# borglab/gtsfm

Hardware: NVIDIA H100
Metric: image_pairs_per_sec (higher is better)
Workload: dtype f32

## Files before the change

gtsfm_b200/_lib.py:

```python
from __future__ import annotations

import ctypes as C
from pathlib import Path
from typing import Optional

import numpy as np

LIB_PATH = Path(__file__).resolve().parent / "libgtsfm_b200.so"

_lib: Optional[C.CDLL] = None


class B200Error(RuntimeError):
    pass


class LightGlueParams(C.Structure):
    _fields_ = [("depth_confidence", C.c_double), ("width_confidence", C.c_double), ("filter_threshold", C.c_double),
                ("prune_min_kpts", C.c_int), ("fp16_attention", C.c_int)]


class LightGluePair(C.Structure):
    _fields_ = [("kp0", C.c_void_p), ("desc0", C.c_void_p), ("n0", C.c_int), ("kp1", C.c_void_p), ("desc1", C.c_void_p), ("n1", C.c_int),
                ("out_matches", C.c_void_p), ("out_scores", C.c_void_p), ("out_k", C.c_int), ("out_stop_layer", C.c_int)]


class MnnPair(C.Structure):
    _fields_ = [("desc0", C.c_void_p), ("n0", C.c_int), ("desc1", C.c_void_p), ("n1", C.c_int), ("out_matches", C.c_void_p),
                ("out_dist", C.c_void_p), ("out_k", C.c_int)]


MNN_ERR_RATIO = -4


class SiftKeypoint(C.Structure):
    _fields_ = [("x", C.c_float), ("y", C.c_float), ("size", C.c_float), ("angle", C.c_float), ("response", C.c_float),
                ("octave", C.c_int32)]


SIFT_KEYPOINT_DTYPE = np.dtype([("x", np.float32), ("y", np.float32), ("size", np.float32), ("angle", np.float32),
                                ("response", np.float32), ("octave", np.int32)])


class SiftImage(C.Structure):
    _fields_ = [("image", C.c_void_p), ("mask", C.c_void_p), ("max_keypoints", C.c_int), ("out_keypoints", C.c_void_p),
                ("out_desc", C.c_void_p), ("out_n", C.c_int), ("out_total", C.c_int)]


SIFT_CAPACITY = -5


class RansacParams(C.Structure):
    _fields_ = [("threshold", C.c_double), ("confidence", C.c_double), ("max_iters", C.c_int), ("seed", C.c_uint64)]


_vp, _i, _f, _sz = C.c_void_p, C.c_int, C.c_float, C.c_size_t
_ip = C.POINTER(C.c_int)

SIGNATURES = {
    "b2_version": (_i, []),
    "b2_create": (_i, [_i, C.POINTER(_vp)]),
    "b2_destroy": (None, [_vp]),
    "b2_last_error": (C.c_char_p, [_vp]),
    "b2_launch_count": (C.c_uint64, [_vp]),
    "b2_h2d_bytes": (C.c_uint64, [_vp]),
    "b2_set_option": (C.c_int, [_vp, C.c_char_p, C.c_int64]),
    "b2_profile_start": (_i, [_vp, C.c_char_p]),
    "b2_profile_stop": (_i, [_vp, C.POINTER(C.c_double), C.POINTER(C.c_uint64), C.POINTER(C.c_double)]),
    "b2_debug_fetch": (C.c_int64, [_vp, C.c_char_p, _vp, C.c_int64]),
    "b2_debug_gemm_host": (_i, [_vp, _i, _vp, _vp, _vp, _vp, _i, _i, _i]),
    "b2_superpoint_set_weights": (_i, [_vp, _vp, _sz]),
    "b2_superpoint_detect_dev": (_i, [_vp, _vp, _i, _i, _i, _sz, _f, _i, _i, _vp, _vp, _i, _ip, C.POINTER(C.c_uint64), _vp]),
    "b2_superpoint_describe_dev": (_i, [_vp, C.c_uint64, _vp, _i, _vp, _vp]),
    "b2_superpoint_extract_dev": (_i, [_vp, _vp, _i, _i, _i, _sz, _f, _i, _i, _i, _vp, _vp, _vp, _ip, _vp]),
    "b2_superpoint_extract_async_dev": (_i, [_vp, _vp, _i, _i, _i, _sz, _f, _i, _i, _i, _vp, _vp, _vp, _vp, _vp]),
    "b2_superpoint_finish_dev": (_i, [_vp, _vp]),
    "b2_topk_indices_dev": (_i, [_vp, _vp, _i, _i, _vp, _ip, _vp]),
    "b2_superpoint_detect_host": (_i, [_vp, _vp, _i, _i, _i, _f, _i, _i, _vp, _vp, _i, _ip, C.POINTER(C.c_uint64)]),
    "b2_superpoint_describe_host": (_i, [_vp, C.c_uint64, _vp, _i, _vp]),
    "b2_image_resize_dev": (_i, [_vp, _vp, _i, _i, _i, _sz, _vp, _i, _i, _vp]),
    "b2_lightglue_set_weights": (_i, [_vp, _vp, _sz]),
    "b2_lightglue_match_dev": (_i, [_vp, _vp, _vp, _i, _vp, _vp, _i, C.POINTER(LightGlueParams), _vp, _vp, _ip, _ip, _vp]),
    "b2_lightglue_match_host": (_i, [_vp, _vp, _vp, _i, _vp, _vp, _i, C.POINTER(LightGlueParams), _vp, _vp, _ip, _ip]),
    "b2_lightglue_match_batched_dev": (_i, [_vp, C.POINTER(LightGluePair), _i, C.POINTER(LightGlueParams), _vp]),
    "b2_superglue_set_weights": (_i, [_vp, _vp, _sz]),
    "b2_superglue_match_dev": (_i, [_vp, _vp, _vp, _vp, _i, _i, _i, _vp, _vp, _vp, _i, _i, _i, _i, _f, _vp, _vp, _ip, _vp]),
    "b2_superglue_match_host": (_i, [_vp, _vp, _vp, _vp, _i, _i, _i, _vp, _vp, _vp, _i, _i, _i, _i, _f, _vp, _vp, _ip]),
    "b2_netvlad_blob_floats": (_sz, []),
    "b2_netvlad_set_weights": (_i, [_vp, _vp, _sz]),
    "b2_netvlad_describe_dev": (_i, [_vp, _vp, _i, _i, _i, _vp, _vp]),
    "b2_netvlad_describe_host": (_i, [_vp, _vp, _i, _i, _i, _vp]),
    "b2_megaloc_blob_floats": (_sz, []),
    "b2_megaloc_set_weights": (_i, [_vp, _vp, _sz]),
    "b2_megaloc_describe_dev": (_i, [_vp, _vp, _i, _i, _i, _vp, _vp]),
    "b2_megaloc_describe_host": (_i, [_vp, _vp, _i, _i, _i, _vp]),
    "b2_megaloc_describe_u8_dev": (_i, [_vp, _vp, _i, _i, _i, _sz, _vp, _vp]),
    "b2_megaloc_resize_u8_dev": (_i, [_vp, _vp, _i, _i, _i, _sz, _vp, _vp]),
    "b2_similarity_pairs_host": (_i, [_vp, _vp, _i, _i, _i, _f, _vp, _vp]),
    "b2_ransac_essential_host": (_i, [_vp, _vp, _vp, _i, C.POINTER(RansacParams), _vp, _vp, _ip, _vp, _vp]),
    "b2_ransac_fundamental_host": (_i, [_vp, _vp, _vp, _i, C.POINTER(RansacParams), _vp, _vp, _ip]),
    "b2_ransac_essential_dev": (_i, [_vp, _vp, _vp, _vp, _i, _vp, _vp, C.POINTER(RansacParams), _vp, _vp, _ip, _vp, _vp, _vp]),
    "b2_recover_pose_host": (_i, [_vp, _vp, _vp, _vp, _i, _vp, _vp, _ip]),
    "b2_mnn_match_batched_dev": (_i, [_vp, C.POINTER(MnnPair), _i, _i, _i, C.c_double, _vp]),
    "b2_mnn_match_host": (_i, [_vp, _vp, _i, _vp, _i, _i, _i, C.c_double, _vp, _vp, _ip]),
    "b2_sift_detect_batched_dev": (_i, [_vp, C.POINTER(SiftImage), _i, _i, _i, _i, _sz, _vp]),
    "b2_sift_detect_host": (_i, [_vp, _vp, _i, _i, _i, _vp, _vp, _vp, _i, _ip]),
}


def load() -> C.CDLL:
    global _lib
    if _lib is not None:
        return _lib
    if not LIB_PATH.exists():
        raise B200Error(f"{LIB_PATH} is missing: run `python -m gtsfm_b200.build` (there is no CPU fallback)")
    lib = C.CDLL(str(LIB_PATH))
    for name, (res, args) in SIGNATURES.items():
        fn = getattr(lib, name)
        fn.restype = res
        fn.argtypes = args
    _lib = lib
    return lib


def ptr(a) -> C.c_void_p:
    if a is None:
        return C.c_void_p(0)
    if isinstance(a, np.ndarray):
        assert a.flags["C_CONTIGUOUS"], "array must be C-contiguous"
        return C.c_void_p(a.ctypes.data)
    if hasattr(a, "data_ptr"):
        assert a.is_contiguous(), "tensor must be contiguous"
        return C.c_void_p(a.data_ptr())
    return C.c_void_p(int(a))


class Context:

    def __init__(self, device: int = 0):
        self._lib = load()
        h = C.c_void_p()
        rc = self._lib.b2_create(int(device), C.byref(h))
        if rc != 0 or not h:
            raise B200Error(
                f"b2_create(device={device}) failed with {rc}: an sm_90 (H100) GPU is required; there is no CPU fallback")
        self.handle = h
        self.device = device

    def check(self, rc: int, what: str) -> None:
        if rc < 0:
            raise B200Error(f"{what} failed ({rc}): {self._lib.b2_last_error(self.handle).decode()}")

    @property
# ... 37 lines not shown
```

gtsfm_b200/csrc/attn_ps.cuh:

```cuda
#pragma once
#include "tma.cuh"

constexpr int AW_Q = 128, AW_KV = 64, AW_D = 64;
constexpr int AW_KV_BYTES = AW_KV * AW_D * 2;
constexpr int AS_NS = 4;
constexpr int AS_HALF = 2 * AW_KV_BYTES;
constexpr int AS_STAGE = 2 * AS_HALF;
constexpr int AS_TILE_BYTES = AS_NS * AS_STAGE;
constexpr int AS_Q_PLANE = AW_Q * AW_D * 2;
constexpr int AS_Q_BYTES = 2 * 2 * AS_Q_PLANE;
constexpr size_t AS_SMEM = AS_TILE_BYTES + AS_Q_BYTES + 1024 + 512;
constexpr int AS_THREADS = 256 + 32;
constexpr float AS_RESCALE = 8.0f;
constexpr int AP_MAXP = 16;

struct AttnPsMaps {
  CUtensorMap kh[AP_MAXP], kl[AP_MAXP], vh[AP_MAXP], vl[AP_MAXP];
};

struct AttnPsProblem {
  const __half *Qh, *Ql;
  __half *Oh, *Ol;
  int Nq, Nk;
  int ldo;
  int qt, tiles;
  int w_end;
  int item0;
};
struct AttnPsArgs {
  AttnPsProblem p[AP_MAXP];
  int nprob;
  float* Opart;
  float* ml;
  int* arrivals;
  int W;
  int quota;
  int max_splits;
  float scale;
  int* err_flag;
};

struct AttnPsSeg {
  int z, item, h, q0, tile0, T, split, nsplits, itemg;
};
__device__ __forceinline__ AttnPsSeg attn_ps_decode(const AttnPsArgs& a, int w, int w_end) {
  AttnPsSeg s;
  s.z = 0;
  while (s.z + 1 < a.nprob && w >= a.p[s.z].w_end) ++s.z;
  const AttnPsProblem& p = a.p[s.z];
  const int base = s.z ? a.p[s.z - 1].w_end : 0;
  const int wl = w - base;
  s.item = wl / p.tiles;
  s.tile0 = wl - s.item * p.tiles;
  s.T = min(p.tiles - s.tile0, w_end - w);
  s.h = s.item / p.qt;
  s.q0 = (s.item - s.h * p.qt) * (2 * AW_Q);
  const int wi0 = base + s.item * p.tiles, wi1 = wi0 + p.tiles;
  const int c_first = wi0 / a.quota;
  s.split = w / a.quota - c_first;
  s.nsplits = (wi1 - 1) / a.quota - c_first + 1;
  s.itemg = p.item0 + s.item;
  return s;
}

template <bool SINGLE>
static __global__ void __launch_bounds__(AS_THREADS, 1) k_flash_ps(const __grid_constant__ AttnPsMaps maps, const __grid_constant__ AttnPsArgs args) {
  extern __shared__ unsigned char ap_raw[];
  const uint32_t raw = tc::smem_u32(ap_raw);
  const uint32_t smem0 = (raw + 1023u) & ~1023u;
  unsigned char* sm = ap_raw + (smem0 - raw);
  uint64_t* bars = reinterpret_cast<uint64_t*>(sm + AS_TILE_BYTES + AS_Q_BYTES);
  uint64_t* kv_full = bars;
  uint64_t* kv_empty = kv_full + AS_NS;
  volatile int* last_flag = reinterpret_cast<volatile int*>(kv_empty + AS_NS);

  const int t = threadIdx.x, warp = t >> 5, lane = t & 31;
  const int w_begin = blockIdx.x * args.quota;
  const int w_end = min(args.W, w_begin + args.quota);

  if (t == 0) {
    for (int i = 0; i < AS_NS; ++i) tc::mbar_init(&kv_full[i], 1), tc::mbar_init(&kv_empty[i], 8);
    tc::fence_mbar_init();
  }
  __syncthreads();
  bool ok = true;

  if (warp == 8) {
    if (lane == 0) {
      int ge = 0;
      for (int w = w_begin; w < w_end;) {
        const AttnPsSeg sg = attn_ps_decode(args, w, w_end);
        const int Nk = args.p[sg.z].Nk;
        for (int e = 0; e < sg.T + 2; ++e) {
          const int g = ge + e, s = g % AS_NS;
          if (g >= AS_NS) ok = tc::mbar_wait(&kv_empty[s], ((g / AS_NS) - 1) & 1) && ok;
          const bool hk = e < sg.T, hv = e >= 2;
          constexpr int PART = SINGLE ? AW_KV_BYTES : AS_HALF;
          tc::mbar_expect_tx(&kv_full[s], (hk ? PART : 0) + (hv ? PART : 0));
          const uint32_t dst = smem0 + s * AS_STAGE;
          if (hk) {
            const int row = sg.h * Nk + (sg.tile0 + e) * AW_KV;
            tc::tma_load_2d(dst, &maps.kh[sg.z], &kv_full[s], 0, row);
            if (!SINGLE) tc::tma_load_2d(dst + AW_KV_BYTES, &maps.kl[sg.z], &kv_full[s], 0, row);
          }
          if (hv) {
            const int row = sg.h * Nk + (sg.tile0 + e - 2) * AW_KV;
            tc::tma_load_2d(dst + AS_HALF, &maps.vh[sg.z], &kv_full[s], 0, row);
            if (!SINGLE) tc::tma_load_2d(dst + AS_HALF + AW_KV_BYTES, &maps.vl[sg.z], &kv_full[s], 0, row);
          }
        }
        ge += sg.T + 2;
        w += sg.T;
      }
    }
  } else {
    const int q = warp >> 2;
    const int r = t & 127;
    const int rq = (warp & 3) * 16 + (lane >> 2);
    const int c2 = (lane & 3) * 2;
    const uint32_t sQ = smem0 + AS_TILE_BYTES + q * 2 * AS_Q_PLANE;
    const float c2s = args.scale * 1.4426950408889634f;
    auto wg_bar = [&]() { asm volatile("bar.sync %0, 128;" ::"r"(1 + q) : "memory"); };
    auto release = [&](int g) { if (lane == 0) tc::mbar_arrive(&kv_empty[g % AS_NS]); };

    int ge = 0;
    for (int w = w_begin; w < w_end;) {
      const AttnPsSeg sg = attn_ps_decode(args, w, w_end);
      const AttnPsProblem& pr = args.p[sg.z];
      const int T = sg.T, Nk = pr.Nk;
      {
        const int qrow = sg.q0 + q * AW_Q + r;
        wg_bar();
#pragma unroll
        for (int pl = 0; pl < (SINGLE ? 1 : 2); ++pl) {
          const __half* src = (pl ? pr.Ql : pr.Qh) + ((size_t)sg.h * pr.Nq + qrow) * 64;
          unsigned char* dst = sm + AS_TILE_BYTES + q * 2 * AS_Q_PLANE + pl * AS_Q_PLANE + r * 128;
#pragma unroll
          for (int c = 0; c < 8; ++c) {
            uint4 v = make_uint4(0u, 0u, 0u, 0u);
            if (qrow < pr.Nq) v = __ldg(reinterpret_cast<const uint4*>(src) + c);
            *reinterpret_cast<uint4*>(dst + ((c ^ (r & 7)) << 4)) = v;
          }
        }
        tc::fence_proxy_async();
        wg_bar();
      }
      float o[2][32];
      float m_ref[2][2], l_i[2][2];
#pragma unroll
      for (int sl = 0; sl < 2; ++sl)
#pragma unroll
        for (int h = 0; h < 2; ++h) m_ref[sl][h] = -INFINITY, l_i[sl][h] = 0.f;
      for (int j = 0; j < 2; ++j) ok = tc::mbar_wait(&kv_full[(ge + j) % AS_NS], ((ge + j) / AS_NS) & 1) && ok;
      if (T == 1) release(ge + 1);
      for (int i = 0; i < T; ++i) {
        const int gv = ge + i + 2;
        ok = tc::mbar_wait(&kv_full[gv % AS_NS], (gv / AS_NS) & 1) && ok;
        const uint32_t sK = smem0 + ((ge + i) % AS_NS) * AS_STAGE, sV = smem0 + (gv % AS_NS) * AS_STAGE + AS_HALF;
        const uint64_t dKh = tc::wg_desc_sw128(sK), dKl = tc::wg_desc_sw128(sK + AW_KV_BYTES);
        const uint64_t dVh = tc::wg_desc_sw128(sV), dVl = tc::wg_desc_sw128(sV + AW_KV_BYTES);
        const int k0 = (sg.tile0 + i) * AW_KV;
#pragma unroll
        for (int sl = 0; sl < 2; ++sl) {
          const uint64_t dQh = tc::wg_desc_sw128(sQ + sl * (64 * 128)), dQl = tc::wg_desc_sw128(sQ + AS_Q_PLANE + sl * (64 * 128));
          float a[32];
          tc::wg_fence();
#pragma unroll
          for (int ks = 0; ks < 4; ++ks) {
            const uint64_t adv = (uint64_t)(ks * 2);
            tc::wg_ss_n64(a, dQh + adv, dKh + adv, ks ? 1u : 0u);
            if (!SINGLE) {
              tc::wg_ss_n64(a, dQh + adv, dKl + adv, 1u);
              tc::wg_ss_n64(a, dQl + adv, dKh + adv, 1u);
            }
          }
          tc::wg_commit();
          tc::wg_wait<0>();
          if (k0 + AW_KV > Nk) {
#pragma unroll
            for (int jj = 0; jj < 32; ++jj)
              if (k0 + 8 * (jj >> 2) + c2 + (jj & 1) >= Nk) a[jj] = -INFINITY;
          }
          uint32_t ph[16], pl[16];
#pragma unroll
          for (int h = 0; h < 2; ++h) {
            float mx = a[2 * h];
#pragma unroll
            for (int j = 0; j < 8; ++j) mx = fmaxf(mx, fmaxf(a[4 * j + 2 * h], a[4 * j + 2 * h + 1]));
            mx = fmaxf(mx, __shfl_xor_sync(0xffffffffu, mx, 1));
            mx = fmaxf(mx, __shfl_xor_sync(0xffffffffu, mx, 2));
            const float m_new = fmaxf(m_ref[sl][h], mx * c2s);
            if (m_new - m_ref[sl][h] > AS_RESCALE) {
              const float corr = tc::ex2(m_ref[sl][h] - m_new);
              l_i[sl][h] *= corr;
              if (i > 0) {
#pragma unroll
                for (int j = 0; j < 8; ++j) o[sl][4 * j + 2 * h] *= corr, o[sl][4 * j + 2 * h + 1] *= corr;
              }
              m_ref[sl][h] = m_new;
            }
            float rs = 0.f;
#pragma unroll
            for (int j = 0; j < 8; ++j) {
              const float p0 = tc::ex2(fmaf(a[4 * j + 2 * h], c2s, -m_ref[sl][h]));
              const float p1 = tc::ex2(fmaf(a[4 * j + 2 * h + 1], c2s, -m_ref[sl][h]));
              rs += p0 + p1;
              const __half2 hh = __floats2half2_rn(p0, p1);
              const int ri = 4 * (j >> 1) + 2 * (j & 1) + h;
              ph[ri] = *reinterpret_cast<const uint32_t*>(&hh);
              if (!SINGLE) {
                const float2 hf = __half22float2(hh);
                const __half2 ll = __floats2half2_rn(p0 - hf.x, p1 - hf.y);
                pl[ri] = *reinterpret_cast<const uint32_t*>(&ll);
              }
            }
            l_i[sl][h] += rs;
          }
          tc::wg_fence();
#pragma unroll
          for (int ks = 0; ks < 4; ++ks) {
            const uint64_t advV = (uint64_t)(ks * 128);
            tc::wg_rs_n64_bt(o[sl], ph + 4 * ks, dVh + advV, (i | ks) ? 1u : 0u);
            if (!SINGLE) {
              tc::wg_rs_n64_bt(o[sl], ph + 4 * ks, dVl + advV, 1u);
              tc::wg_rs_n64_bt(o[sl], pl + 4 * ks, dVh + advV, 1u);
            }
          }
          tc::wg_commit();
          tc::wg_wait<0>();
        }
        release(ge + i);
        if (i + 2 >= T) release(gv);
      }
      ge += T + 2;
      w += T;
#pragma unroll
      for (int sl = 0; sl < 2; ++sl)
#pragma unroll
        for (int h = 0; h < 2; ++h) {
          l_i[sl][h] += __shfl_xor_sync(0xffffffffu, l_i[sl][h], 1);
          l_i[sl][h] += __shfl_xor_sync(0xffffffffu, l_i[sl][h], 2);
        }
      auto write_row = [&](const float* v, float inv, int qrow) {
        uint32_t* dh = reinterpret_cast<uint32_t*>(pr.Oh + (size_t)qrow * pr.ldo + sg.h * 64 + c2);
        uint32_t* dl = reinterpret_cast<uint32_t*>(pr.Ol + (size_t)qrow * pr.ldo + sg.h * 64 + c2);
#pragma unroll
        for (int j = 0; j < 8; ++j) {
          uint32_t hi, lo;
          if (SINGLE) {
            const __half2 hh = __floats2half2_rn(tc::clamp_h(v[4 * j] * inv), tc::clamp_h(v[4 * j + 1] * inv));
            hi = *reinterpret_cast<const uint32_t*>(&hh), lo = 0u;
          } else {
            tc::split2(v[4 * j] * inv, v[4 * j + 1] * inv, hi, lo);
          }
          dh[4 * j] = hi;
          dl[4 * j] = lo;
        }
      };
      if (sg.nsplits == 1) {
#pragma unroll
        for (int sl = 0; sl < 2; ++sl)
#pragma unroll
          for (int h = 0; h < 2; ++h) {
            const int qrow = sg.q0 + q * AW_Q + sl * 64 + rq + 8 * h;
            if (qrow >= pr.Nq) continue;
            float v[32];
#pragma unroll
            for (int j = 0; j < 8; ++j) v[4 * j] = o[sl][4 * j + 2 * h], v[4 * j + 1] = o[sl][4 * j + 2 * h + 1];
            write_row(v, 1.0f / l_i[sl][h], qrow);
          }
      } else {
        const size_t slot0 = (size_t)sg.itemg * args.max_splits;
#pragma unroll
        for (int sl = 0; sl < 2; ++sl)
#pragma unroll
          for (int h = 0; h < 2; ++h) {
            const int rl = q * AW_Q + sl * 64 + rq + 8 * h;
            if (sg.q0 + rl >= pr.Nq) continue;
            const size_t rowi = (slot0 + sg.split) * 256 + rl;
            float* dst = args.Opart + rowi * 64 + c2;
#pragma unroll
            for (int j = 0; j < 8; ++j) *reinterpret_cast<float2*>(dst + 8 * j) = make_float2(o[sl][4 * j + 2 * h], o[sl][4 * j + 2 * h + 1]);
            if (c2 == 0) *reinterpret_cast<float2*>(args.ml + rowi * 2) = make_float2(m_ref[sl][h], l_i[sl][h]);
          }
        __threadfence();
        wg_bar();
        if (r == 0) {
          int* cnt = args.arrivals + sg.itemg * 2 + q;
          const int old = atomicAdd(cnt, 1);
          const int last = old == sg.nsplits - 1;
          if (last) atomicExch(cnt, 0);
          last_flag[q] = last;
        }
        wg_bar();
        if (last_flag[q]) {
          __threadfence();
#pragma unroll 1
          for (int sl = 0; sl < 2; ++sl)
#pragma unroll 1
            for (int h = 0; h < 2; ++h) {
              const int rl = q * AW_Q + sl * 64 + rq + 8 * h;
              const int qrow = sg.q0 + rl;
              if (qrow >= pr.Nq) continue;
              float m = -INFINITY;
              for (int sp = 0; sp < sg.nsplits; ++sp) m = fmaxf(m, __ldcg(args.ml + ((slot0 + sp) * 256 + rl) * 2));
              float l = 0.f, v[32];
#pragma unroll
              for (int j = 0; j < 32; ++j) v[j] = 0.f;
              for (int sp = 0; sp < sg.nsplits; ++sp) {
                const size_t ri = (slot0 + sp) * 256 + rl;
                const float2 mlv = __ldcg(reinterpret_cast<const float2*>(args.ml + ri * 2));
                const float wgt = tc::ex2(mlv.x - m);
                l = fmaf(mlv.y, wgt, l);
                const float* src = args.Opart + ri * 64 + c2;
// ... 15 lines not shown
```

gtsfm_b200/csrc/debug.cu:

```cuda
#include <stdlib.h>

#include "common.cuh"
#include "linear.cuh"

extern "C" int b2_debug_gemm_host(b2_context* ctx, int mode, const float* A, const float* B, const float* bias, float* C,
                                  int M, int N, int K) {
  if (!ctx || !A || !B || !C || M <= 0 || N <= 0 || K <= 0 || (K % 64)) return B2_ERR_ARG;
  std::lock_guard<std::mutex> lk(ctx->mu);
  cudaSetDevice(ctx->device);
  cudaStream_t st = ctx->stream;
  DevBuf dA, dB, dC, dBias, dBh, dBl, dErr;
  B2_CUDA(ctx, dA.ensure((size_t)M * K * 4));
  B2_CUDA(ctx, dB.ensure((size_t)N * K * 4));
  B2_CUDA(ctx, dC.ensure((size_t)M * N * 4));
  B2_CUDA(ctx, dBias.ensure((size_t)N * 4));
  B2_CUDA(ctx, dErr.ensure(16));
  B2_CUDA(ctx, cudaMemcpyAsync(dA.p, A, (size_t)M * K * 4, cudaMemcpyHostToDevice, st));
  B2_CUDA(ctx, cudaMemcpyAsync(dB.p, B, (size_t)N * K * 4, cudaMemcpyHostToDevice, st));
  if (bias) B2_CUDA(ctx, cudaMemcpyAsync(dBias.p, bias, (size_t)N * 4, cudaMemcpyHostToDevice, st));
  B2_CUDA(ctx, cudaMemsetAsync(dErr.p, 0, 16, st));
  int rc = B2_OK;
  if (mode == 0) {
    rc = launch_gemm(ctx, st, gemm_linear(dA.as<float>(), K, K, dB.as<float>(), bias ? dBias.as<float>() : nullptr, dC.as<float>(), N, M, N));
  } else {
    DevBuf dAh, dAl;
    B2_CUDA(ctx, dAh.ensure((size_t)M * K * 2));
    B2_CUDA(ctx, dAl.ensure((size_t)M * K * 2));
    B2_CUDA(ctx, dBh.ensure((size_t)N * K * 2));
    B2_CUDA(ctx, dBl.ensure((size_t)N * K * 2));
    B2_LAUNCH(ctx, k_split_f32, (unsigned)(((size_t)M * K + 255) / 256), 256, 0, st, dA.as<float>(), (size_t)M * K, dAh.as<__half>(), dAl.as<__half>());
    B2_LAUNCH(ctx, k_split_f32, (unsigned)(((size_t)N * K + 255) / 256), 256, 0, st, dB.as<float>(), (size_t)N * K, dBh.as<__half>(), dBl.as<__half>());
    B2_CUDA(ctx, cudaFuncSetAttribute(k_gemm_ws, cudaFuncAttributeMaxDynamicSharedMemorySize, (int)GW_SMEM));
    TcWeights tw{nullptr, nullptr, nullptr, dErr.as<int>(), true};
    tw.sm_count = ctx->sm_count;
    LinArgs a;
    a.a1p = {dAh.as<__half>(), dAl.as<__half>()}, a.lda1 = K, a.K1 = K, a.bp = {dBh.as<__half>(), dBl.as<__half>()}, a.ldb = K;
    a.bias = bias ? dBias.as<float>() : nullptr, a.cf = dC.as<float>(), a.ldc = N, a.tc_want_f32 = true, a.M = M, a.N = N;
    rc = run_linear(ctx, st, tw, &a, 1);
    if (rc == B2_OK) {
      cudaError_t e = cudaStreamSynchronize(st);
      if (e != cudaSuccess) rc = b2_fail(ctx, B2_ERR_CUDA, std::string("debug gemm: ") + cudaGetErrorString(e));
    }
    dAh.release(), dAl.release();
  }
  int err = 0;
  if (rc == B2_OK) {
    cudaError_t e = cudaMemcpyAsync(C, dC.p, (size_t)M * N * 4, cudaMemcpyDeviceToHost, st);
    if (e == cudaSuccess) e = cudaMemcpyAsync(&err, dErr.p, 4, cudaMemcpyDeviceToHost, st);
    if (e == cudaSuccess) e = cudaStreamSynchronize(st);
    if (e != cudaSuccess) rc = b2_fail(ctx, B2_ERR_CUDA, std::string("debug gemm: ") + cudaGetErrorString(e));
  }
  dA.release(), dB.release(), dC.release(), dBias.release(), dBh.release(), dBl.release(), dErr.release();
  if (rc == B2_OK && err) rc = b2_fail(ctx, B2_ERR_STATE, "wgmma pipeline timed out on an mbarrier (kernel bug)");
  return rc;
}
```

gtsfm_b200/csrc/tc.cuh:

```cuda
#pragma once
#include <cuda_fp16.h>
#include <stdint.h>

namespace tc {

__device__ __forceinline__ uint32_t smem_u32(const void* p) { return (uint32_t)__cvta_generic_to_shared(p); }

__device__ __forceinline__ void mbar_init(uint64_t* bar, uint32_t count) {
  asm volatile("mbarrier.init.shared::cta.b64 [%0], %1;" ::"r"(smem_u32(bar)), "r"(count) : "memory");
}
__device__ __forceinline__ void fence_mbar_init() { asm volatile("fence.mbarrier_init.release.cluster;" ::: "memory"); }
__device__ __forceinline__ void fence_proxy_async() { asm volatile("fence.proxy.async.shared::cta;" ::: "memory"); }
__device__ __forceinline__ void mbar_arrive(uint64_t* bar) {
  asm volatile("mbarrier.arrive.shared::cta.b64 _, [%0];" ::"r"(smem_u32(bar)) : "memory");
}
__device__ __forceinline__ bool mbar_wait(uint64_t* bar, uint32_t parity) {
  const uint32_t addr = smem_u32(bar);
  for (uint32_t spin = 0; spin < (1u << 24); ++spin) {
    uint32_t ok;
    asm volatile(
        "{\n\t.reg .pred p;\n\t"
        "mbarrier.try_wait.parity.shared::cta.b64 p, [%1], %2;\n\t"
        "selp.u32 %0, 1, 0, p;\n\t}"
        : "=r"(ok)
        : "r"(addr), "r"(parity)
        : "memory");
    if (ok) return true;
  }
  return false;
}

__device__ __forceinline__ uint64_t wg_desc_sw128(uint32_t saddr, uint32_t sbo_bytes = 1024) {
  uint64_t d = 0;
  d |= (uint64_t)((saddr >> 4) & 0x3FFF);
  d |= (uint64_t)1 << 16;
  d |= (uint64_t)((sbo_bytes >> 4) & 0x3FFF) << 32;
  d |= (uint64_t)1 << 62;
  return d;
}
__device__ __forceinline__ void wg_fence() { asm volatile("wgmma.fence.sync.aligned;" ::: "memory"); }
__device__ __forceinline__ void wg_commit() { asm volatile("wgmma.commit_group.sync.aligned;" ::: "memory"); }
template <int N>
__device__ __forceinline__ void wg_wait() {
  asm volatile("wgmma.wait_group.sync.aligned %0;" ::"n"(N) : "memory");
}
__device__ __forceinline__ void wg_ss_n128(float* d, uint64_t adesc, uint64_t bdesc, uint32_t scale_d) {
  asm volatile(
      "{\n\t.reg .pred p;\n\t"
      "setp.ne.b32 p, %66, 0;\n\t"
      "wgmma.mma_async.sync.aligned.m64n128k16.f32.f16.f16 {%0, %1, %2, %3, %4, %5, %6, %7, %8, %9, %10, %11, %12, %13, %14, %15, %16, %17, %18, %19, %20, %21, %22, %23, %24, %25, %26, %27, %28, %29, %30, %31, %32, %33, %34, %35, %36, %37, %38, %39, %40, %41, %42, %43, %44, %45, %46, %47, %48, %49, %50, %51, %52, %53, %54, %55, %56, %57, %58, %59, %60, %61, %62, %63}, %64, %65, p, 1, 1, 0, 0;\n\t}"
      : "+f"(d[0]), "+f"(d[1]), "+f"(d[2]), "+f"(d[3]), "+f"(d[4]), "+f"(d[5]), "+f"(d[6]), "+f"(d[7]), "+f"(d[8]), "+f"(d[9]), "+f"(d[10]), "+f"(d[11]), "+f"(d[12]), "+f"(d[13]), "+f"(d[14]), "+f"(d[15]), "+f"(d[16]), "+f"(d[17]), "+f"(d[18]), "+f"(d[19]), "+f"(d[20]), "+f"(d[21]), "+f"(d[22]), "+f"(d[23]), "+f"(d[24]), "+f"(d[25]), "+f"(d[26]), "+f"(d[27]), "+f"(d[28]), "+f"(d[29]), "+f"(d[30]), "+f"(d[31]), "+f"(d[32]), "+f"(d[33]), "+f"(d[34]), "+f"(d[35]), "+f"(d[36]), "+f"(d[37]), "+f"(d[38]), "+f"(d[39]), "+f"(d[40]), "+f"(d[41]), "+f"(d[42]), "+f"(d[43]), "+f"(d[44]), "+f"(d[45]), "+f"(d[46]), "+f"(d[47]), "+f"(d[48]), "+f"(d[49]), "+f"(d[50]), "+f"(d[51]), "+f"(d[52]), "+f"(d[53]), "+f"(d[54]), "+f"(d[55]), "+f"(d[56]), "+f"(d[57]), "+f"(d[58]), "+f"(d[59]), "+f"(d[60]), "+f"(d[61]), "+f"(d[62]), "+f"(d[63])
      : "l"(adesc), "l"(bdesc), "r"(scale_d)
      : "memory");
}
__device__ __forceinline__ void wg_ss_n64(float* d, uint64_t adesc, uint64_t bdesc, uint32_t scale_d) {
  asm volatile(
      "{\n\t.reg .pred p;\n\t"
      "setp.ne.b32 p, %34, 0;\n\t"
      "wgmma.mma_async.sync.aligned.m64n64k16.f32.f16.f16 {%0, %1, %2, %3, %4, %5, %6, %7, %8, %9, %10, %11, %12, %13, %14, %15, %16, %17, %18, %19, %20, %21, %22, %23, %24, %25, %26, %27, %28, %29, %30, %31}, %32, %33, p, 1, 1, 0, 0;\n\t}"
      : "+f"(d[0]), "+f"(d[1]), "+f"(d[2]), "+f"(d[3]), "+f"(d[4]), "+f"(d[5]), "+f"(d[6]), "+f"(d[7]), "+f"(d[8]), "+f"(d[9]), "+f"(d[10]), "+f"(d[11]), "+f"(d[12]), "+f"(d[13]), "+f"(d[14]), "+f"(d[15]), "+f"(d[16]), "+f"(d[17]), "+f"(d[18]), "+f"(d[19]), "+f"(d[20]), "+f"(d[21]), "+f"(d[22]), "+f"(d[23]), "+f"(d[24]), "+f"(d[25]), "+f"(d[26]), "+f"(d[27]), "+f"(d[28]), "+f"(d[29]), "+f"(d[30]), "+f"(d[31])
      : "l"(adesc), "l"(bdesc), "r"(scale_d)
      : "memory");
}
__device__ __forceinline__ void wg_ss_u8_n128(uint32_t* d, uint64_t adesc, uint64_t bdesc, uint32_t scale_d) {
  asm volatile(
      "{\n\t.reg .pred p;\n\t"
      "setp.ne.b32 p, %66, 0;\n\t"
      "wgmma.mma_async.sync.aligned.m64n128k32.s32.u8.u8 {%0, %1, %2, %3, %4, %5, %6, %7, %8, %9, %10, %11, %12, %13, %14, %15, %16, %17, %18, %19, %20, %21, %22, %23, %24, %25, %26, %27, %28, %29, %30, %31, %32, %33, %34, %35, %36, %37, %38, %39, %40, %41, %42, %43, %44, %45, %46, %47, %48, %49, %50, %51, %52, %53, %54, %55, %56, %57, %58, %59, %60, %61, %62, %63}, %64, %65, p;\n\t}"
      : "+r"(d[0]), "+r"(d[1]), "+r"(d[2]), "+r"(d[3]), "+r"(d[4]), "+r"(d[5]), "+r"(d[6]), "+r"(d[7]), "+r"(d[8]), "+r"(d[9]), "+r"(d[10]), "+r"(d[11]), "+r"(d[12]), "+r"(d[13]), "+r"(d[14]), "+r"(d[15]), "+r"(d[16]), "+r"(d[17]), "+r"(d[18]), "+r"(d[19]), "+r"(d[20]), "+r"(d[21]), "+r"(d[22]), "+r"(d[23]), "+r"(d[24]), "+r"(d[25]), "+r"(d[26]), "+r"(d[27]), "+r"(d[28]), "+r"(d[29]), "+r"(d[30]), "+r"(d[31]), "+r"(d[32]), "+r"(d[33]), "+r"(d[34]), "+r"(d[35]), "+r"(d[36]), "+r"(d[37]), "+r"(d[38]), "+r"(d[39]), "+r"(d[40]), "+r"(d[41]), "+r"(d[42]), "+r"(d[43]), "+r"(d[44]), "+r"(d[45]), "+r"(d[46]), "+r"(d[47]), "+r"(d[48]), "+r"(d[49]), "+r"(d[50]), "+r"(d[51]), "+r"(d[52]), "+r"(d[53]), "+r"(d[54]), "+r"(d[55]), "+r"(d[56]), "+r"(d[57]), "+r"(d[58]), "+r"(d[59]), "+r"(d[60]), "+r"(d[61]), "+r"(d[62]), "+r"(d[63])
      : "l"(adesc), "l"(bdesc), "r"(scale_d)
      : "memory");
}
__device__ __forceinline__ void wg_rs_n64_bt(float* d, const uint32_t* a, uint64_t bdesc, uint32_t scale_d) {
  asm volatile(
      "{\n\t.reg .pred p;\n\t"
      "setp.ne.b32 p, %37, 0;\n\t"
      "wgmma.mma_async.sync.aligned.m64n64k16.f32.f16.f16 {%0, %1, %2, %3, %4, %5, %6, %7, %8, %9, %10, %11, %12, %13, %14, %15, %16, %17, %18, %19, %20, %21, %22, %23, %24, %25, %26, %27, %28, %29, %30, %31}, {%32, %33, %34, %35}, %36, p, 1, 1, 1;\n\t}"
      : "+f"(d[0]), "+f"(d[1]), "+f"(d[2]), "+f"(d[3]), "+f"(d[4]), "+f"(d[5]), "+f"(d[6]), "+f"(d[7]), "+f"(d[8]), "+f"(d[9]), "+f"(d[10]), "+f"(d[11]), "+f"(d[12]), "+f"(d[13]), "+f"(d[14]), "+f"(d[15]), "+f"(d[16]), "+f"(d[17]), "+f"(d[18]), "+f"(d[19]), "+f"(d[20]), "+f"(d[21]), "+f"(d[22]), "+f"(d[23]), "+f"(d[24]), "+f"(d[25]), "+f"(d[26]), "+f"(d[27]), "+f"(d[28]), "+f"(d[29]), "+f"(d[30]), "+f"(d[31])
      : "r"(a[0]), "r"(a[1]), "r"(a[2]), "r"(a[3]), "l"(bdesc), "r"(scale_d)
      : "memory");
}

__device__ __forceinline__ void cp_async16(uint32_t dst_smem, const void* src, uint32_t src_bytes) {
  asm volatile("cp.async.cg.shared.global [%0], [%1], 16, %2;" ::"r"(dst_smem), "l"(src), "r"(src_bytes) : "memory");
}
__device__ __forceinline__ void cp_async_commit() { asm volatile("cp.async.commit_group;" ::: "memory"); }
template <int N>
__device__ __forceinline__ void cp_async_wait() {
  asm volatile("cp.async.wait_group %0;" ::"n"(N) : "memory");
}

constexpr float LO_SCALE = 2048.0f;
constexpr float LO_INV = 1.0f / 2048.0f;
constexpr float H_MAX = 65504.0f;
__device__ __forceinline__ float clamp_h(float x) { return fminf(fmaxf(x, -H_MAX), H_MAX); }
__device__ __forceinline__ void split_h(float x, __half& hi, __half& lo) {
  x = clamp_h(x);
  hi = __float2half_rn(x);
  lo = __float2half_rn((x - __half2float(hi)) * LO_SCALE);
}
__device__ __forceinline__ void split_h_unscaled(float x, __half& hi, __half& lo) {
  x = clamp_h(x);
  hi = __float2half_rn(x);
  lo = __float2half_rn(x - __half2float(hi));
}
__device__ __forceinline__ void split8(const float* x, uint4& hi, uint4& lo) {
  __half h[8], l[8];
#pragma unroll
  for (int i = 0; i < 8; ++i) split_h(x[i], h[i], l[i]);
  hi = *reinterpret_cast<uint4*>(h);
  lo = *reinterpret_cast<uint4*>(l);
}
__device__ __forceinline__ float ex2(float x) {
  float y;
  asm("ex2.approx.ftz.f32 %0, %1;" : "=f"(y) : "f"(x));
  return y;
}
__device__ __forceinline__ void split2(float a, float b, uint32_t& hi, uint32_t& lo) {
  a = clamp_h(a), b = clamp_h(b);
  const __half2 h = __floats2half2_rn(a, b);
  const float2 hf = __half22float2(h);
  const __half2 l = __floats2half2_rn((a - hf.x) * LO_SCALE, (b - hf.y) * LO_SCALE);
  hi = *reinterpret_cast<const uint32_t*>(&h);
  lo = *reinterpret_cast<const uint32_t*>(&l);
}
__device__ __forceinline__ void split2_unscaled(float a, float b, uint32_t& hi, uint32_t& lo) {
  const __half2 h = __floats2half2_rn(a, b);
  const float2 hf = __half22float2(h);
  const __half2 l = __floats2half2_rn(a - hf.x, b - hf.y);
  hi = *reinterpret_cast<const uint32_t*>(&h);
  lo = *reinterpret_cast<const uint32_t*>(&l);
}
__device__ __forceinline__ void split2_unscaled_clamped(float a, float b, uint32_t& hi, uint32_t& lo) {
  split2_unscaled(clamp_h(a), clamp_h(b), hi, lo);
}
}
```

include/gtsfm_b200.h:

```cpp
#ifndef GTSFM_B200_H
#define GTSFM_B200_H

#include <stddef.h>
#include <stdint.h>

#ifdef __cplusplus
extern "C" {
#endif

typedef struct b2_context b2_context;

int b2_version(void);
int b2_create(int device, b2_context** out);
void b2_destroy(b2_context* ctx);
const char* b2_last_error(const b2_context* ctx);
uint64_t b2_launch_count(const b2_context* ctx);
uint64_t b2_h2d_bytes(const b2_context* ctx);
int b2_set_option(b2_context* ctx, const char* name, int64_t value);
int b2_profile_start(b2_context* ctx, const char* kernel_prefix);
int b2_profile_stop(b2_context* ctx, double* total_ms, uint64_t* launches, double* work);
int64_t b2_debug_fetch(b2_context* ctx, const char* name, float* host_out, int64_t max_floats);

int b2_debug_gemm_host(b2_context* ctx, int mode, const float* A, const float* B, const float* bias, float* C, int M, int N,
                       int K);

int b2_superpoint_set_weights(b2_context* ctx, const float* host_blob, size_t n_floats);

int b2_superpoint_detect_dev(b2_context* ctx, const uint8_t* image, int height, int width, int channels, size_t pitch,
                             float keypoint_threshold, int nms_radius, int border, float* out_xy, float* out_score,
                             int cap, int* out_n, uint64_t* out_map_token, void* stream);
int b2_superpoint_describe_dev(b2_context* ctx, uint64_t map_token, const float* xy, int n, float* out_desc, void* stream);
int b2_superpoint_extract_dev(b2_context* ctx, const uint8_t* image, int height, int width, int channels, size_t pitch,
                              float keypoint_threshold, int nms_radius, int border, int max_keypoints, float* out_xy,
                              float* out_score, float* out_desc, int* out_n, void* stream);
int b2_superpoint_extract_async_dev(b2_context* ctx, const uint8_t* image, int height, int width, int channels, size_t pitch,
                                    float threshold, int nms_radius, int border, int max_keypoints, float* out_xy,
                                    float* out_score, float* out_desc, int* out_n_pinned, void* stream);
int b2_superpoint_finish_dev(b2_context* ctx, void* stream);
int b2_topk_indices_dev(b2_context* ctx, const float* scores, int n, int k, int32_t* out_idx, int* out_k, void* stream);

int b2_superpoint_detect_host(b2_context* ctx, const uint8_t* image, int height, int width, int channels,
                              float keypoint_threshold, int nms_radius, int border, float* out_xy, float* out_score,
                              int cap, int* out_n, uint64_t* out_map_token);
int b2_superpoint_describe_host(b2_context* ctx, uint64_t map_token, const float* xy, int n, float* out_desc);

int b2_image_resize_dev(b2_context* ctx, const uint8_t* src, int height, int width, int channels, size_t pitch, uint8_t* dst,
                        int new_height, int new_width, void* stream);

int b2_lightglue_set_weights(b2_context* ctx, const float* host_blob, size_t n_floats);

typedef struct b2_lightglue_params {
  double depth_confidence;
  double width_confidence;
  double filter_threshold;
  int prune_min_kpts;
  int fp16_attention;
} b2_lightglue_params;

int b2_lightglue_match_dev(b2_context* ctx, const float* kp0, const float* desc0, int n0, const float* kp1,
                           const float* desc1, int n1, const b2_lightglue_params* params, int64_t* out_matches,
                           float* out_scores, int* out_k, int* out_stop_layer, void* stream);
int b2_lightglue_match_host(b2_context* ctx, const float* kp0, const float* desc0, int n0, const float* kp1,
                            const float* desc1, int n1, const b2_lightglue_params* params, int64_t* out_matches,
                            float* out_scores, int* out_k, int* out_stop_layer);

typedef struct b2_lightglue_pair {
  const float* kp0;
  const float* desc0;
  int n0;
  const float* kp1;
  const float* desc1;
  int n1;
  int64_t* out_matches;
  float* out_scores;
  int out_k;
  int out_stop_layer;
} b2_lightglue_pair;
int b2_lightglue_match_batched_dev(b2_context* ctx, b2_lightglue_pair* pairs, int n_pairs, const b2_lightglue_params* params,
                                   void* stream);

int b2_superglue_set_weights(b2_context* ctx, const float* host_blob, size_t n_floats);
int b2_superglue_match_dev(b2_context* ctx, const float* kp0, const float* score0, const float* desc0, int n0, int h0,
                           int w0, const float* kp1, const float* score1, const float* desc1, int n1, int h1, int w1,
                           int sinkhorn_iters, float match_threshold, uint32_t* out_matches, float* out_scores,
                           int* out_k, void* stream);
int b2_superglue_match_host(b2_context* ctx, const float* kp0, const float* score0, const float* desc0, int n0, int h0,
                            int w0, const float* kp1, const float* score1, const float* desc1, int n1, int h1, int w1,
                            int sinkhorn_iters, float match_threshold, uint32_t* out_matches, float* out_scores,
                            int* out_k);

typedef struct b2_ransac_params {
  double threshold;
  double confidence;
  int max_iters;
  uint64_t seed;
} b2_ransac_params;

int b2_ransac_essential_host(b2_context* ctx, const double* x1, const double* x2, int k, const b2_ransac_params* params,
                             double* out_model, uint8_t* out_mask, int* out_num_inliers, double* out_R, double* out_t);
int b2_ransac_fundamental_host(b2_context* ctx, const double* x1, const double* x2, int k,
                               const b2_ransac_params* params, double* out_model, uint8_t* out_mask,
                               int* out_num_inliers);
int b2_ransac_essential_dev(b2_context* ctx, const float* kp1, const float* kp2, const int64_t* matches, int k,
                            const double* cal1, const double* cal2, const b2_ransac_params* params, double* out_model,
                            uint8_t* out_mask_dev, int* out_num_inliers, double* out_R, double* out_t, void* stream);
int b2_recover_pose_host(b2_context* ctx, const double* E, const double* x1, const double* x2, int k, double* out_R,
                         double* out_t, int* out_num_good);
// ... 54 lines not shown
```

Baseline: 85.54.

## Overlap QK and PV wgmma across two query slices in flash attention kernel

Restructures the flash attention consumer loop so the QK^T wgmma for both query slices is issued together, and one slice's softmax runs while the other slice's matrix multiplies are still in flight. The Q high plane is loaded into registers and fed to register-sourced wgmma. Producer warps are widened to a full warpgroup that gives up registers via setmaxnreg so the consumers can hold more. It also adds a host debug entry point for testing attention. The price is higher register pressure and a risk of spills or occupancy loss.

```diff
diff --git a/gtsfm_b200/_lib.py b/gtsfm_b200/_lib.py
--- a/gtsfm_b200/_lib.py
+++ b/gtsfm_b200/_lib.py
@@ -69,6 +69,7 @@
     "b2_profile_stop": (_i, [_vp, C.POINTER(C.c_double), C.POINTER(C.c_uint64), C.POINTER(C.c_double)]),
     "b2_debug_fetch": (C.c_int64, [_vp, C.c_char_p, _vp, C.c_int64]),
     "b2_debug_gemm_host": (_i, [_vp, _i, _vp, _vp, _vp, _vp, _i, _i, _i]),
+    "b2_debug_attention_host": (_i, [_vp, _i, _ip, _ip, _i, _f, _i, _vp, _vp, _vp, _vp]),
     "b2_superpoint_set_weights": (_i, [_vp, _vp, _sz]),
     "b2_superpoint_detect_dev": (_i, [_vp, _vp, _i, _i, _i, _sz, _f, _i, _i, _vp, _vp, _i, _ip, C.POINTER(C.c_uint64), _vp]),
     "b2_superpoint_describe_dev": (_i, [_vp, C.c_uint64, _vp, _i, _vp, _vp]),
diff --git a/gtsfm_b200/csrc/attn_ps.cuh b/gtsfm_b200/csrc/attn_ps.cuh
--- a/gtsfm_b200/csrc/attn_ps.cuh
+++ b/gtsfm_b200/csrc/attn_ps.cuh
@@ -10,7 +10,7 @@
 constexpr int AS_Q_PLANE = AW_Q * AW_D * 2;
 constexpr int AS_Q_BYTES = 2 * 2 * AS_Q_PLANE;
 constexpr size_t AS_SMEM = AS_TILE_BYTES + AS_Q_BYTES + 1024 + 512;
-constexpr int AS_THREADS = 256 + 32;
+constexpr int AS_THREADS = 256 + 128;
 constexpr float AS_RESCALE = 8.0f;
 constexpr int AP_MAXP = 16;
 
@@ -85,8 +85,9 @@
   __syncthreads();
   bool ok = true;
 
-  if (warp == 8) {
-    if (lane == 0) {
+  if (warp >= 8) {
+    asm volatile("setmaxnreg.dec.sync.aligned.u32 24;\n" ::: "memory");
+    if (warp == 8 && lane == 0) {
       int ge = 0;
       for (int w = w_begin; w < w_end;) {
         const AttnPsSeg sg = attn_ps_decode(args, w, w_end);
@@ -114,6 +115,7 @@
       }
     }
   } else {
+    asm volatile("setmaxnreg.inc.sync.aligned.u32 240;\n" ::: "memory");
     const int q = warp >> 2;
     const int r = t & 127;
     const int rq = (warp & 3) * 16 + (lane >> 2);
@@ -145,91 +147,117 @@
         tc::fence_proxy_async();
         wg_bar();
       }
+      uint32_t qf[2][16];
+#pragma unroll
+      for (int sl = 0; sl < 2; ++sl)
+#pragma unroll
+        for (int h = 0; h < 2; ++h) {
+          const int qrow = sg.q0 + q * AW_Q + sl * 64 + rq + 8 * h;
+          const uint32_t* src = reinterpret_cast<const uint32_t*>(pr.Qh + ((size_t)sg.h * pr.Nq + qrow) * 64 + c2);
+#pragma unroll
+          for (int j = 0; j < 8; ++j) qf[sl][4 * (j >> 1) + 2 * (j & 1) + h] = qrow < pr.Nq ? __ldg(src + 4 * j) : 0u;
+        }
       float o[2][32];
       float m_ref[2][2], l_i[2][2];
 #pragma unroll
       for (int sl = 0; sl < 2; ++sl)
 #pragma unroll
         for (int h = 0; h < 2; ++h) m_ref[sl][h] = -INFINITY, l_i[sl][h] = 0.f;
+      float s[2][32];
+      uint32_t ph[2][16], pl[2][16];
+      auto qk = [&](int i, int sl) {
+        const uint32_t sK = smem0 + ((ge + i) % AS_NS) * AS_STAGE;
+        const uint64_t dKh = tc::wg_desc_sw128(sK), dKl = tc::wg_desc_sw128(sK + AW_KV_BYTES);
+        const uint64_t dQl = tc::wg_desc_sw128(sQ + AS_Q_PLANE + sl * (64 * 128));
+        tc::wg_fence();
+#pragma unroll
+        for (int ks = 0; ks < 4; ++ks) {
+          const uint64_t adv = (uint64_t)(ks * 2);
+          tc::wg_rs_n64(s[sl], qf[sl] + 4 * ks, dKh + adv, ks ? 1u : 0u);
+          if (!SINGLE) {
+            tc::wg_rs_n64(s[sl], qf[sl] + 4 * ks, dKl + adv, 1u);
+            tc::wg_ss_n64(s[sl], dQl + adv, dKh + adv, 1u);
+          }
+        }
+        tc::wg_commit();
+      };
+      auto softmax = [&](int i, int sl) {
+        float* a = s[sl];
+        const int k0 = (sg.tile0 + i) * AW_KV;
+        if (k0 + AW_KV > Nk) {
+#pragma unroll
+          for (int jj = 0; jj < 32; ++jj)
+            if (k0 + 8 * (jj >> 2) + c2 + (jj & 1) >= Nk) a[jj] = -INFINITY;
+        }
+#pragma unroll
+        for (int h = 0; h < 2; ++h) {
+          float mx = a[2 * h];
+#pragma unroll
+          for (int j = 0; j < 8; ++j) mx = fmaxf(mx, fmaxf(a[4 * j + 2 * h], a[4 * j + 2 * h + 1]));
+          mx = fmaxf(mx, __shfl_xor_sync(0xffffffffu, mx, 1));
+          mx = fmaxf(mx, __shfl_xor_sync(0xffffffffu, mx, 2));
+          const float m_new = fmaxf(m_ref[sl][h], mx * c2s);
+          if (m_new - m_ref[sl][h] > AS_RESCALE) {
+            const float corr = tc::ex2(m_ref[sl][h] - m_new);
+            l_i[sl][h] *= corr;
+            if (i > 0) {
+#pragma unroll
+              for (int j = 0; j < 8; ++j) o[sl][4 * j + 2 * h] *= corr, o[sl][4 * j + 2 * h + 1] *= corr;
+            }
+            m_ref[sl][h] = m_new;
+          }
+          float rs = 0.f;
+#pragma unroll
+          for (int j = 0; j < 8; ++j) {
+            const float p0 = tc::ex2(fmaf(a[4 * j + 2 * h], c2s, -m_ref[sl][h]));
+            const float p1 = tc::ex2(fmaf(a[4 * j + 2 * h + 1], c2s, -m_ref[sl][h]));
+            rs += p0 + p1;
+            const __half2 hh = __floats2half2_rn(p0, p1);
+            const int ri = 4 * (j >> 1) + 2 * (j & 1) + h;
+            ph[sl][ri] = *reinterpret_cast<const uint32_t*>(&hh);
+            if (!SINGLE) {
+              const float2 hf = __half22float2(hh);
+              const __half2 ll = __floats2half2_rn(p0 - hf.x, p1 - hf.y);
+              pl[sl][ri] = *reinterpret_cast<const uint32_t*>(&ll);
+            }
+          }
+          l_i[sl][h] += rs;
+        }
+      };
+      auto pv = [&](int i, int sl) {
+        const uint32_t sV = smem0 + ((ge + i + 2) % AS_NS) * AS_STAGE + AS_HALF;
+        const uint64_t dVh = tc::wg_desc_sw128(sV), dVl = tc::wg_desc_sw128(sV + AW_KV_BYTES);
+        tc::wg_fence();
+#pragma unroll
+        for (int ks = 0; ks < 4; ++ks) {
+          const uint64_t advV = (uint64_t)(ks * 128);
+          tc::wg_rs_n64_bt(o[sl], ph[sl] + 4 * ks, dVh + advV, (i | ks) ? 1u : 0u);
+          if (!SINGLE) {
+            tc::wg_rs_n64_bt(o[sl], ph[sl] + 4 * ks, dVl + advV, 1u);
+            tc::wg_rs_n64_bt(o[sl], pl[sl] + 4 * ks, dVh + advV, 1u);
+          }
+        }
+        tc::wg_commit();
+      };
+
       for (int j = 0; j < 2; ++j) ok = tc::mbar_wait(&kv_full[(ge + j) % AS_NS], ((ge + j) / AS_NS) & 1) && ok;
       if (T == 1) release(ge + 1);
       for (int i = 0; i < T; ++i) {
+        qk(i, 0);
+        qk(i, 1);
+        tc::wg_wait<1>();
+        tc::fence_regs(s[0]);
+        softmax(i, 0);
         const int gv = ge + i + 2;
         ok = tc::mbar_wait(&kv_full[gv % AS_NS], (gv / AS_NS) & 1) && ok;
-        const uint32_t sK = smem0 + ((ge + i) % AS_NS) * AS_STAGE, sV = smem0 + (gv % AS_NS) * AS_STAGE + AS_HALF;
-        const uint64_t dKh = tc::wg_desc_sw128(sK), dKl = tc::wg_desc_sw128(sK + AW_KV_BYTES);
-        const uint64_t dVh = tc::wg_desc_sw128(sV), dVl = tc::wg_desc_sw128(sV + AW_KV_BYTES);
-        const int k0 = (sg.tile0 + i) * AW_KV;
-#pragma unroll
-        for (int sl = 0; sl < 2; ++sl) {
-          const uint64_t dQh = tc::wg_desc_sw128(sQ + sl * (64 * 128)), dQl = tc::wg_desc_sw128(sQ + AS_Q_PLANE + sl * (64 * 128));
-          float a[32];
-          tc::wg_fence();
-#pragma unroll
-          for (int ks = 0; ks < 4; ++ks) {
-            const uint64_t adv = (uint64_t)(ks * 2);
-            tc::wg_ss_n64(a, dQh + adv, dKh + adv, ks ? 1u : 0u);
-            if (!SINGLE) {
-              tc::wg_ss_n64(a, dQh + adv, dKl + adv, 1u);
-              tc::wg_ss_n64(a, dQl + adv, dKh + adv, 1u);
-            }
-          }
-          tc::wg_commit();
-          tc::wg_wait<0>();
-          if (k0 + AW_KV > Nk) {
-#pragma unroll
-            for (int jj = 0; jj < 32; ++jj)
-              if (k0 + 8 * (jj >> 2) + c2 + (jj & 1) >= Nk) a[jj] = -INFINITY;
-          }
-          uint32_t ph[16], pl[16];
-#pragma unroll
-          for (int h = 0; h < 2; ++h) {
-            float mx = a[2 * h];
-#pragma unroll
-            for (int j = 0; j < 8; ++j) mx = fmaxf(mx, fmaxf(a[4 * j + 2 * h], a[4 * j + 2 * h + 1]));
-            mx = fmaxf(mx, __shfl_xor_sync(0xffffffffu, mx, 1));
-            mx = fmaxf(mx, __shfl_xor_sync(0xffffffffu, mx, 2));
-            const float m_new = fmaxf(m_ref[sl][h], mx * c2s);
-            if (m_new - m_ref[sl][h] > AS_RESCALE) {
-              const float corr = tc::ex2(m_ref[sl][h] - m_new);
-              l_i[sl][h] *= corr;
-              if (i > 0) {
-#pragma unroll
-                for (int j = 0; j < 8; ++j) o[sl][4 * j + 2 * h] *= corr, o[sl][4 * j + 2 * h + 1] *= corr;
-              }
-              m_ref[sl][h] = m_new;
-            }
-            float rs = 0.f;
-#pragma unroll
-            for (int j = 0; j < 8; ++j) {
-              const float p0 = tc::ex2(fmaf(a[4 * j + 2 * h], c2s, -m_ref[sl][h]));
-              const float p1 = tc::ex2(fmaf(a[4 * j + 2 * h + 1], c2s, -m_ref[sl][h]));
-              rs += p0 + p1;
-              const __half2 hh = __floats2half2_rn(p0, p1);
-              const int ri = 4 * (j >> 1) + 2 * (j & 1) + h;
-              ph[ri] = *reinterpret_cast<const uint32_t*>(&hh);
-              if (!SINGLE) {
-                const float2 hf = __half22float2(hh);
-                const __half2 ll = __floats2half2_rn(p0 - hf.x, p1 - hf.y);
-                pl[ri] = *reinterpret_cast<const uint32_t*>(&ll);
-              }
-            }
-            l_i[sl][h] += rs;
-          }
-          tc::wg_fence();
-#pragma unroll
-          for (int ks = 0; ks < 4; ++ks) {
-            const uint64_t advV = (uint64_t)(ks * 128);
-            tc::wg_rs_n64_bt(o[sl], ph + 4 * ks, dVh + advV, (i | ks) ? 1u : 0u);
-            if (!SINGLE) {
-              tc::wg_rs_n64_bt(o[sl], ph + 4 * ks, dVl + advV, 1u);
-              tc::wg_rs_n64_bt(o[sl], pl + 4 * ks, dVh + advV, 1u);
-            }
-          }
-          tc::wg_commit();
-          tc::wg_wait<0>();
-        }
+        pv(i, 0);
+        tc::wg_wait<1>();
+        tc::fence_regs(s[1]);
         release(ge + i);
+        softmax(i, 1);
+        pv(i, 1);
+        tc::wg_wait<0>();
+        tc::fence_regs(o[0]), tc::fence_regs(o[1]);
         if (i + 2 >= T) release(gv);
       }
       ge += T + 2;
diff --git a/gtsfm_b200/csrc/debug.cu b/gtsfm_b200/csrc/debug.cu
--- a/gtsfm_b200/csrc/debug.cu
+++ b/gtsfm_b200/csrc/debug.cu
@@ -1,7 +1,14 @@
 #include <stdlib.h>
+
+#include <vector>
 
 #include "common.cuh"
 #include "linear.cuh"
+
+static __global__ void k_split_unscaled_f32(const float* __restrict__ x, size_t n, __half* __restrict__ hi, __half* __restrict__ lo) {
+  const size_t i = (size_t)blockIdx.x * blockDim.x + threadIdx.x;
+  if (i < n) tc::split_h_unscaled(x[i], hi[i], lo[i]);
+}
 
 extern "C" int b2_debug_gemm_host(b2_context* ctx, int mode, const float* A, const float* B, const float* bias, float* C,
                                   int M, int N, int K) {
@@ -54,3 +61,54 @@
   if (rc == B2_OK && err) rc = b2_fail(ctx, B2_ERR_STATE, "wgmma pipeline timed out on an mbarrier (kernel bug)");
   return rc;
 }
+
+extern "C" int b2_debug_attention_host(b2_context* ctx, int np, const int* nq, const int* nk, int heads, float scale, int single,
+                                       const float* q, const float* k, const float* v, float* o) {
+  if (!ctx || !nq || !nk || !q || !k || !v || !o || np <= 0 || np > AP_MAXP || heads <= 0) return B2_ERR_ARG;
+  size_t eq = 0, ek = 0;
+  for (int z = 0; z < np; ++z) {
+    if (nq[z] <= 0 || nk[z] <= 0) return B2_ERR_ARG;
+    eq += (size_t)nq[z] * heads * 64, ek += (size_t)nk[z] * heads * 64;
+  }
+  std::lock_guard<std::mutex> lk(ctx->mu);
+  cudaSetDevice(ctx->device);
+  cudaStream_t st = ctx->stream;
+  const size_t n = eq + 2 * ek;
+  DevBuf dIn, dPl, dO, dErr, part, ml, cnt;
+  B2_CUDA(ctx, dIn.ensure(n * 4));
+  B2_CUDA(ctx, dPl.ensure(n * 2 * 2));
+  B2_CUDA(ctx, dO.ensure(eq * 2 * 2));
+  B2_CUDA(ctx, dErr.ensure(16));
+  float* in = dIn.as<float>();
+  B2_CUDA(ctx, cudaMemcpyAsync(in, q, eq * 4, cudaMemcpyHostToDevice, st));
+  B2_CUDA(ctx, cudaMemcpyAsync(in + eq, k, ek * 4, cudaMemcpyHostToDevice, st));
+  B2_CUDA(ctx, cudaMemcpyAsync(in + eq + ek, v, ek * 4, cudaMemcpyHostToDevice, st));
+  B2_CUDA(ctx, cudaMemsetAsync(dErr.p, 0, 16, st));
+  __half *hi = dPl.as<__half>(), *lo = hi + n, *oh = dO.as<__half>(), *ol = oh + eq;
+  B2_LAUNCH(ctx, k_split_unscaled_f32, (unsigned)((n + 255) / 256), 256, 0, st, in, n, hi, lo);
+  B2_CUDA(ctx, cudaFuncSetAttribute(k_flash_ps<false>, cudaFuncAttributeMaxDynamicSharedMemorySize, (int)AS_SMEM));
+  B2_CUDA(ctx, cudaFuncSetAttribute(k_flash_ps<true>, cudaFuncAttributeMaxDynamicSharedMemorySize, (int)AS_SMEM));
+  FlashPlanes fp[AP_MAXP];
+  size_t qo = 0, ko = eq;
+  for (int z = 0; z < np; ++z) {
+    const size_t vo = ko + ek;
+    fp[z] = {{hi + qo, lo + qo}, {hi + ko, lo + ko}, {hi + vo, lo + vo}, {oh + qo, ol + qo}, nq[z], nk[z], heads, 64 * heads};
+    qo += (size_t)nq[z] * heads * 64, ko += (size_t)nk[z] * heads * 64;
+  }
+  TcWeights tw{nullptr, nullptr, nullptr, dErr.as<int>(), true};
+  tw.attn_part = &part, tw.attn_ml = &ml, tw.attn_cnt = &cnt, tw.sm_count = ctx->sm_count;
+  int rc = run_flash_planes(ctx, st, tw, fp, np, scale, single != 0);
+  std::vector<__half> ho(2 * eq);
+  int err = 0;
+  if (rc == B2_OK) {
+    cudaError_t e = cudaMemcpyAsync(ho.data(), oh, eq * 2 * 2, cudaMemcpyDeviceToHost, st);
+    if (e == cudaSuccess) e = cudaMemcpyAsync(&err, dErr.p, 4, cudaMemcpyDeviceToHost, st);
+    if (e == cudaSuccess) e = cudaStreamSynchronize(st);
+    if (e != cudaSuccess) rc = b2_fail(ctx, B2_ERR_CUDA, std::string("debug attention: ") + cudaGetErrorString(e));
+  }
+  if (rc == B2_OK)
+    for (size_t i = 0; i < eq; ++i) o[i] = __half2float(ho[i]) + __half2float(ho[eq + i]) * tc::LO_INV;
+  dIn.release(), dPl.release(), dO.release(), dErr.release(), part.release(), ml.release(), cnt.release();
+  if (rc == B2_OK && err) rc = b2_fail(ctx, B2_ERR_STATE, "wgmma attention timed out on an mbarrier (kernel bug)");
+  return rc;
+}
diff --git a/gtsfm_b200/csrc/tc.cuh b/gtsfm_b200/csrc/tc.cuh
--- a/gtsfm_b200/csrc/tc.cuh
+++ b/gtsfm_b200/csrc/tc.cuh
@@ -44,6 +44,10 @@
 __device__ __forceinline__ void wg_wait() {
   asm volatile("wgmma.wait_group.sync.aligned %0;" ::"n"(N) : "memory");
 }
+__device__ __forceinline__ void fence_regs(float* r) {
+#pragma unroll
+  for (int j = 0; j < 32; ++j) asm volatile("" : "+f"(r[j])::"memory");
+}
 __device__ __forceinline__ void wg_ss_n128(float* d, uint64_t adesc, uint64_t bdesc, uint32_t scale_d) {
   asm volatile(
       "{\n\t.reg .pred p;\n\t"
@@ -69,6 +73,15 @@
       "wgmma.mma_async.sync.aligned.m64n128k32.s32.u8.u8 {%0, %1, %2, %3, %4, %5, %6, %7, %8, %9, %10, %11, %12, %13, %14, %15, %16, %17, %18, %19, %20, %21, %22, %23, %24, %25, %26, %27, %28, %29, %30, %31, %32, %33, %34, %35, %36, %37, %38, %39, %40, %41, %42, %43, %44, %45, %46, %47, %48, %49, %50, %51, %52, %53, %54, %55, %56, %57, %58, %59, %60, %61, %62, %63}, %64, %65, p;\n\t}"
       : "+r"(d[0]), "+r"(d[1]), "+r"(d[2]), "+r"(d[3]), "+r"(d[4]), "+r"(d[5]), "+r"(d[6]), "+r"(d[7]), "+r"(d[8]), "+r"(d[9]), "+r"(d[10]), "+r"(d[11]), "+r"(d[12]), "+r"(d[13]), "+r"(d[14]), "+r"(d[15]), "+r"(d[16]), "+r"(d[17]), "+r"(d[18]), "+r"(d[19]), "+r"(d[20]), "+r"(d[21]), "+r"(d[22]), "+r"(d[23]), "+r"(d[24]), "+r"(d[25]), "+r"(d[26]), "+r"(d[27]), "+r"(d[28]), "+r"(d[29]), "+r"(d[30]), "+r"(d[31]), "+r"(d[32]), "+r"(d[33]), "+r"(d[34]), "+r"(d[35]), "+r"(d[36]), "+r"(d[37]), "+r"(d[38]), "+r"(d[39]), "+r"(d[40]), "+r"(d[41]), "+r"(d[42]), "+r"(d[43]), "+r"(d[44]), "+r"(d[45]), "+r"(d[46]), "+r"(d[47]), "+r"(d[48]), "+r"(d[49]), "+r"(d[50]), "+r"(d[51]), "+r"(d[52]), "+r"(d[53]), "+r"(d[54]), "+r"(d[55]), "+r"(d[56]), "+r"(d[57]), "+r"(d[58]), "+r"(d[59]), "+r"(d[60]), "+r"(d[61]), "+r"(d[62]), "+r"(d[63])
       : "l"(adesc), "l"(bdesc), "r"(scale_d)
+      : "memory");
+}
+__device__ __forceinline__ void wg_rs_n64(float* d, const uint32_t* a, uint64_t bdesc, uint32_t scale_d) {
+  asm volatile(
+      "{\n\t.reg .pred p;\n\t"
+      "setp.ne.b32 p, %37, 0;\n\t"
+      "wgmma.mma_async.sync.aligned.m64n64k16.f32.f16.f16 {%0, %1, %2, %3, %4, %5, %6, %7, %8, %9, %10, %11, %12, %13, %14, %15, %16, %17, %18, %19, %20, %21, %22, %23, %24, %25, %26, %27, %28, %29, %30, %31}, {%32, %33, %34, %35}, %36, p, 1, 1, 0;\n\t}"
+      : "+f"(d[0]), "+f"(d[1]), "+f"(d[2]), "+f"(d[3]), "+f"(d[4]), "+f"(d[5]), "+f"(d[6]), "+f"(d[7]), "+f"(d[8]), "+f"(d[9]), "+f"(d[10]), "+f"(d[11]), "+f"(d[12]), "+f"(d[13]), "+f"(d[14]), "+f"(d[15]), "+f"(d[16]), "+f"(d[17]), "+f"(d[18]), "+f"(d[19]), "+f"(d[20]), "+f"(d[21]), "+f"(d[22]), "+f"(d[23]), "+f"(d[24]), "+f"(d[25]), "+f"(d[26]), "+f"(d[27]), "+f"(d[28]), "+f"(d[29]), "+f"(d[30]), "+f"(d[31])
+      : "r"(a[0]), "r"(a[1]), "r"(a[2]), "r"(a[3]), "l"(bdesc), "r"(scale_d)
       : "memory");
 }
 __device__ __forceinline__ void wg_rs_n64_bt(float* d, const uint32_t* a, uint64_t bdesc, uint32_t scale_d) {
diff --git a/include/gtsfm_b200.h b/include/gtsfm_b200.h
--- a/include/gtsfm_b200.h
+++ b/include/gtsfm_b200.h
@@ -23,6 +23,8 @@
 
 int b2_debug_gemm_host(b2_context* ctx, int mode, const float* A, const float* B, const float* bias, float* C, int M, int N,
                        int K);
+int b2_debug_attention_host(b2_context* ctx, int np, const int* nq, const int* nk, int heads, float scale, int single,
+                            const float* q, const float* k, const float* v, float* o);
 
 int b2_superpoint_set_weights(b2_context* ctx, const float* host_blob, size_t n_floats);
 
```

New measurement: 88.77, median of 6. 3.8% higher.
